# google-research/frame-interpolation

Hardware: AMD Instinct MI355X
Metric: interpolated frames/sec @1080p (higher is better)
Workload: dtype f32; 1 GPU; 1080p_2x2: 1920x1080 pair, align 64, block_shape [2, 2] -> 4 tile(s) of 960x576 in one batch, film_net published config, seeded synthetic weights, t=0.5; parallelism=1 independent GPU(s), weights RCCL-broadcast once, exec=direct launches, two lanes, lanes=1

## Files before the change

frame-interpolation_amd/csrc/conv_igemm.hip:

```cpp
#include "conv_buf_impl.h"
#include "conv_wino43_impl.h"
#include "conv_wino2d_impl.h"
#include "conv_fold4_impl.h"
#include "conv_c3_impl.h"
#ifdef FILM_EXTRA_FAMILIES
#include "conv_halo_impl.h"
#include "conv_split_impl.h"
#include "conv_wino_impl.h"
#include "conv_winox3_impl.h"
#include "conv_foldx3_impl.h"
#endif

template <int F>
static hipError_t launch_shape(const ConvParams& p, int shape, hipStream_t s) {
  switch (shape) {
    case TILE_128x128: return conv_buf_launch<128, 128, 2, 2, F>(p, s);
    case TILE_256x64: return conv_buf_launch<256, 64, 4, 1, F>(p, s);
    case TILE_256x32: return conv_buf_launch<256, 32, 4, 1, F>(p, s);
    case TILE_64x64: return conv_buf_launch<64, 64, 2, 2, F>(p, s);
    case TILE_128x32: return conv_buf_launch<128, 32, 4, 1, F>(p, s);
    case TILE_128x64: return conv_buf_launch<128, 64, 2, 2, F>(p, s);
    case TILE_256x128: return conv_buf_launch<256, 128, 4, 2, F>(p, s);
    default: return hipErrorInvalidValue;
  }
// ... 33 lines not shown

template <int F>
static hipError_t launch_wino(const ConvParams& p, int shape, hipStream_t s) {
  switch (shape) {
    case WINO_4x128: return conv_wino_launch<4, 128, 4, 2, F>(p, s);
    case WINO_4x64: return conv_wino_launch<4, 64, 4, 1, F>(p, s);
    case WINO_4x128_W16: return conv_wino_launch<4, 128, 4, 4, F>(p, s);
    case WINO_4x32: return conv_wino_launch<4, 32, 4, 1, F>(p, s);
    case WINO_8x64_W16: return conv_wino_launch<8, 64, 8, 2, F>(p, s);
    case WINO_8x32_W8: return conv_wino_launch<8, 32, 8, 1, F>(p, s);
    case WINO_2x64: return conv_wino_launch<2, 64, 2, 2, F>(p, s);
    case WINO_4x64_W8: return conv_wino_launch<4, 64, 4, 2, F>(p, s);
    default: return hipErrorInvalidValue;
  }
}

#endif

template <int F>
static hipError_t launch_wino43(const ConvParams& p, int shape, hipStream_t s) {
  switch (shape) {
    case W43_Q16_4x64_T21_P2: return conv_wino43_launch<4, 64, 2, 1, F | W43_F_PF2, 16>(p, s);
    case W43_Q16_4x32_T11_P2: return conv_wino43_launch<4, 32, 1, 1, F | W43_F_PF2, 16>(p, s);
    case W43_Q16_4x64_N1_P2: return conv_wino43_launch<4, 64, 1, 1, F | W43_F_PF2, 16, 1>(p, s);
    case W43_Q8_8x64_T21_P2: return conv_wino43_launch<8, 64, 2, 1, F | W43_F_PF2, 8>(p, s);
    case W43_Q8_8x64_N1_P2: return conv_wino43_launch<8, 64, 1, 1, F | W43_F_PF2, 8, 1>(p, s);
    case W43_Q8_8x32_T11_BG: return conv_wino43_launch<8, 32, 1, 1, F | W43_F_BG, 8>(p, s);
    case W43_Q8_8x32_T11_P2: return conv_wino43_launch<8, 32, 1, 1, F | W43_F_PF2, 8>(p, s);
#ifdef FILM_EXTRA_FAMILIES
    case W43_4x64_T21: return conv_wino43_launch<4, 64, 2, 1, F>(p, s);
    case W43_4x64_T12: return conv_wino43_launch<4, 64, 1, 2, F>(p, s);
    case W43_4x32_T11: return conv_wino43_launch<4, 32, 1, 1, F>(p, s);
    case W43_Q16_4x64_T21: return conv_wino43_launch<4, 64, 2, 1, F, 16>(p, s);
    case W43_Q16_4x64_T12: return conv_wino43_launch<4, 64, 1, 2, F, 16>(p, s);
    case W43_Q16_4x32_T11: return conv_wino43_launch<4, 32, 1, 1, F, 16>(p, s);
    case W43_Q16_4x64_N1: return conv_wino43_launch<4, 64, 1, 1, F, 16, 1>(p, s);
    case W43_Q16_4x64_T12_P2: return conv_wino43_launch<4, 64, 1, 2, F | W43_F_PF2, 16>(p, s);
    case W43_Q16_4x32_T11_BG: return conv_wino43_launch<4, 32, 1, 1, F | W43_F_BG, 16>(p, s);
    case W43_Q8_8x64_T12_P2: return conv_wino43_launch<8, 64, 1, 2, F | W43_F_PF2, 8>(p, s);
#endif
    default: return hipErrorInvalidValue;
  }
}

template <int F>
static hipError_t launch_wino2d(const ConvParams& p, int shape, hipStream_t s) {
  switch (shape) {
    case W2D_8x64: return conv_wino2d_launch_any<64, F>(p, s);
    case W2D_8x32: return conv_wino2d_launch_any<32, F>(p, s);
    case W2D_8x32_S2: return conv_wino2d_launch_any<32, F, 2>(p, s);
    case W2D_16x64: return conv_wino2d_launch_any<64, F | W2D_F_SQ>(p, s);
    case W2D_16x32: return conv_wino2d_launch_any<32, F | W2D_F_SQ>(p, s);
    case W2D_16x32_S2: return conv_wino2d_launch_any<32, F | W2D_F_SQ, 2>(p, s);
    default: return hipErrorInvalidValue;
  }
}

template <int F>
static hipError_t launch_fold4(const ConvParams& p, int shape, hipStream_t s) {
  switch (shape) {
    case F4_4x64: return conv_fold4_launch<2, F>(p, s);
    case F4_4x32: return conv_fold4_launch<1, F>(p, s);
    default: return hipErrorInvalidValue;
  }
}

#ifdef FILM_EXTRA_FAMILIES
template <int F>
static hipError_t launch_winox3(const ConvParams& p, int shape, hipStream_t s) {
  switch (shape) {
    case WX3_4x128_T22: return conv_winox3_launch<4, 128, 2, 2, F>(p, s);
    case WX3_4x64_T12: return conv_winox3_launch<4, 64, 1, 2, F>(p, s);
    case WX3_4x64_T21: return conv_winox3_launch<4, 64, 2, 1, F>(p, s);
    case WX3_4x32_T11: return conv_winox3_launch<4, 32, 1, 1, F>(p, s);
    default: return hipErrorInvalidValue;
  }
}

template <int F>
static hipError_t launch_foldx3(const ConvParams& p, int shape, hipStream_t s) {
  switch (shape) {
    case FX3_4x64: return conv_foldx3_launch<4, 64, 4, 1, F>(p, s);
    case FX3_8x64: return conv_foldx3_launch<8, 64, 8, 1, F>(p, s);
    case FX3_4x128: return conv_foldx3_launch<4, 128, 4, 2, F>(p, s);
    default: return hipErrorInvalidValue;
  }
}
#endif


__global__ __launch_bounds__(256) void conv_splitk_reduce_kernel(const float* __restrict__ part, const float* __restrict__ bias,
                                                                 float* __restrict__ out, int M, int Cout, int ostride,
                                                                 int S, int leaky) {
  const int G = Cout >> 2;
  const unsigned idx = blockIdx.x * 256u + threadIdx.x;
  if (idx >= (unsigned)M * (unsigned)G) return;
  const unsigned m = idx / (unsigned)G, g = idx - m * (unsigned)G;
  const size_t plane = (size_t)M * Cout;
  const float4* src = reinterpret_cast<const float4*>(part + (size_t)m * Cout + g * 4);
  float4 a = *reinterpret_cast<const float4*>(bias + g * 4);
  for (int sidx = 0; sidx < S; ++sidx) {
    const float4 v = src[(size_t)sidx * (plane >> 2)];
    a.x += v.x; a.y += v.y; a.z += v.z; a.w += v.w;
  }
  if (leaky) {
    a.x = a.x > 0.f ? a.x : 0.2f * a.x; a.y = a.y > 0.f ? a.y : 0.2f * a.y;
// ... 60 lines not shown
```

frame-interpolation_amd/csrc/conv_wino2d_impl.h:

```cpp
#pragma once
#include "conv_common.h"

enum { W2D_F_SQ = 128,
       W2D_F_XEPI = 8,
       W2D_DBG_TIME = 8192 };


template <bool SQ> struct W2dSlotTable { unsigned v[24 * 64]; };
template <bool SQ> constexpr W2dSlotTable<SQ> w2d_make_slot_table() {
  constexpr int QW = SQ ? 4 : 8, TH = SQ ? 16 : 8, HR = TH + 2, PW = 4 * QW + 2;
  constexpr int CO4 = (PW + 3) / 4, MO4 = 4 * CO4, RP4 = 4 * MO4 + (SQ ? 2 : 4);
  W2dSlotTable<SQ> t{};
  for (int sl = 0; sl < 24 * 64; ++sl) {
    const int r = sl / RP4, rem = sl % RP4, m = rem / MO4, rr = rem % MO4, c = rr / CO4, k = rr % CO4, px = 4 * k + m;
    const bool ok = r < HR && rem < 4 * MO4 && px < PW;
    t.v[sl] = ok ? ((unsigned)r << 24 | (unsigned)px << 8 | (unsigned)c << 4) : 0xFFFFFFFFu;
  }
  return t;
}
template <bool SQ> __device__ const W2dSlotTable<SQ> w2d_slot_table = w2d_make_slot_table<SQ>();

template <int BN, int FLAGS, int NS_ = 3>
__global__ __launch_bounds__(4 * (BN / 32) * 64, (BN == 32) ? 2 : 1) void conv_wino2d_kernel(ConvParams p) {
  constexpr bool SQ = (FLAGS & W2D_F_SQ) != 0;
  constexpr int QW = SQ ? 4 : 8, TH = SQ ? 16 : 8, HR = TH + 2, PXW = 4 * QW, PW = PXW + 2;
  static_assert(QW * (TH / 2) == 32, "32 units per tile");
  constexpr int NG = BN / 32, NW = 4 * NG;
  constexpr int CO4 = (PW + 3) / 4, MO4 = 4 * CO4, RP4 = 4 * MO4 + (SQ ? 2 : 4);
  constexpr int NREQ = 24;
  constexpr int STAGE4 = NREQ * 64;
  constexpr int NS = NS_;
  static_assert(NS == 2 || NS == 3, "stages");
  constexpr int IPW = NREQ / NW;
  static_assert(NREQ % NW == 0, "requests per wave");
  static_assert(HR * RP4 <= STAGE4, "stage size");
  constexpr bool XE = (FLAGS & W2D_F_XEPI) != 0;
  constexpr unsigned OOB = 0xFFFFFFFFu;

  extern __shared__ __attribute__((aligned(1024))) float smem[];

  const int t = threadIdx.x;
  const int lane = t & 63;
  const int wv = __builtin_amdgcn_readfirstlane(t >> 6);
  const int l31 = lane & 31, half = lane >> 5;
  const int mu = wv & 3, ng = wv >> 2;

  unsigned long long tm0 = 0, tm1 = 0, tm2 = 0, tmA = 0, tmB = 0, tmC = 0, tmW = 0, tmE1 = 0, tmE2 = 0, tmE3 = 0;
  unsigned long long rt0 = 0;
  if constexpr ((FLAGS & W2D_DBG_TIME) != 0) { rt0 = __builtin_amdgcn_s_memrealtime(); tm0 = __builtin_readcyclecounter(); }

  int aH = p.H, aW = p.W, aNB = p.NB, aCtot = p.Ctot, aKsplit = p.ksplit, aNseg = p.nseg, aUnused = p.unused_chain;
  unsigned a_tpi = p.mg_tpi, a_ntx = p.mg_ntx, a_nby = p.mg_nby;
  int ntx_ = p.tl_ntx, tpi_ = p.tl_tpi;
  int aGx = (int)gridDim.x, aGy = (int)gridDim.y;
  const float* aS0ptr = p.seg[0].ptr;
  int aS0stride = p.seg[0].stride, aS0C = p.seg[0].C, aS0boff = p.seg[0].boff, aS0bmod = p.seg[0].bmod;
  const float* aWptr = p.w;
  unsigned rtab[(24 / (4 * (BN / 32)))];
#pragma unroll
  for (int n = 0; n < 24 / NW; ++n) rtab[n] = w2d_slot_table<SQ>.v[t + 64 * NW * n];
  {
    unsigned long long q0 = (unsigned long long)(uintptr_t)aS0ptr, q1 = (unsigned long long)(uintptr_t)aWptr;
    asm volatile("" : "+s"(aH), "+s"(aW), "+s"(aNB), "+s"(aCtot), "+s"(aKsplit), "+s"(aNseg), "+s"(aUnused), "+s"(a_tpi), "+s"(a_ntx), "+s"(a_nby), "+s"(ntx_), "+s"(tpi_),
                      "+s"(aGx), "+s"(aGy), "+s"(q0), "+s"(q1), "+s"(aS0stride), "+s"(aS0C), "+s"(aS0boff), "+s"(aS0bmod));
    aS0ptr = reinterpret_cast<const float*>((uintptr_t)q0);
    aWptr = reinterpret_cast<const float*>((uintptr_t)q1);
  }
  unsigned long long tmK = 0, tmT = 0;
  if constexpr ((FLAGS & W2D_DBG_TIME) != 0) tmK = __builtin_readcyclecounter();
  int bx = blockIdx.x, by = blockIdx.y;
  if constexpr ((FLAGS & CONV_B_XCD_M) != 0) {
    const int nbx = aGx, nby = aGy;
    const int nwg = nbx * nby;
    const int lin = by * nbx + bx;
    const int xcd = lin & 7, idx = lin >> 3;
    const int q = nwg >> 3, r = nwg & 7;
    const int base = xcd < r ? xcd * (q + 1) : r * (q + 1) + (xcd - r) * q;
    const int nl = base + idx;
    bx = (int)conv_udiv((unsigned)nl, a_nby);
    by = nl - bx * nby;
  }
  const int ntx = ntx_, tpi = tpi_;
  const int img = (int)conv_udiv((unsigned)bx, a_tpi);
  const int trow0 = (int)conv_udiv((unsigned)(bx - img * tpi), a_ntx);
  const int y0 = trow0 * TH, x0 = (bx - img * tpi - trow0 * ntx) * PXW;
  const int n0 = by * BN;

  unsigned rvoff[IPW];
  int rsg = 0, rc0 = 0, rsegC = 0;
// ... 36 lines not shown
      rvoff[n] = tv == OOB ? OOB : off;
    }
  };
  auto raw_setup_seg = [&]() {
    const ConvSeg& s = p.seg[rsg];
    raw_setup_seg_of(s.ptr, s.stride, s.C, s.boff, s.bmod);
  };
  auto dma_piece = [&](int n, int stage) {
    const unsigned so = (unsigned)rc0 * 4u;
    const unsigned base = lds0 + (unsigned)stage * (STAGE4 * 16u) + (unsigned)(wv + NW * n) * 1024u;
    asm volatile("s_mov_b32 m0, %0\n\ts_nop 0\n\tbuffer_load_dwordx4 %1, %2, %3 offen lds" ::"s"(base), "v"(rvoff[n]), "s"(rrsrc), "s"(so)
                 : "memory");
  };
  auto dma_advance = [&]() {
    rc0 += 16;
    if (rc0 >= rsegC) {
      if (rsg + 1 < aNseg) { rc0 = 0; ++rsg; raw_setup_seg(); }
    }
  };
  const int ksp = XE && aKsplit > 1 ? aKsplit : 1;
  const int nsc_all = aCtot >> 4;
  int sc0 = 0, sc1 = nsc_all;
  if (ksp > 1) {
    sc0 = (int)((unsigned)nsc_all * blockIdx.z / (unsigned)ksp);
    sc1 = (int)((unsigned)nsc_all * (blockIdx.z + 1u) / (unsigned)ksp);
    int c = sc0 * 16;
    while (rsg + 1 < aNseg && c >= p.seg[rsg].C) { c -= p.seg[rsg].C; ++rsg; }
    rc0 = c;
  }
  auto raw_issue = [&](int stage) {
#pragma unroll
    for (int n = 0; n < IPW; ++n) dma_piece(n, stage);
    dma_advance();
  };

  const int nkc = aCtot / 8, nsc = sc1 - sc0, kc0 = 2 * sc0, kc1 = 2 * sc1;
  const conv_rsrc_t brsrc = conv_make_rsrc(conv_uniform_ptr(aWptr));
  const unsigned bvoff = (unsigned)((half * 32 + l31) * 16);
  const int ct = n0 / 32 + ng;
  auto slab = [&](int kc) { return (unsigned)(((ct * nkc + (kc < nkc ? kc : nkc - 1)) * 4 + mu) * 6) * 1024u; };
  bf4 fbg[2][6];

  f32x16 acc[6];

  const bf4* const smem4 = reinterpret_cast<const bf4*>(smem);
  const int ur = l31 / QW, lq = l31 % QW;
  const int ra = mu == 0 ? 0 : mu == 2 ? 2 : 1, rb = mu == 0 ? 2 : mu == 1 ? 2 : mu == 2 ? 1 : 3;
  const float sgn = mu == 1 ? 1.f : -1.f;
  const int ix_a = (2 * ur + ra) * RP4 + half * CO4 + lq, ix_b = (2 * ur + rb) * RP4 + half * CO4 + lq;
  typedef float f2 __attribute__((ext_vector_type(2)));
  f2 A[2][6][2];
  bf4 d[6];
  bf4 d2[6];

  using C0 = std::integral_constant<int, 0>;
  using C1 = std::integral_constant<int, 1>;
  auto read_row = [&](bf4 (&dst)[6], int ix, int stage, auto h_c) {
    constexpr int IMM = decltype(h_c)::value * 2 * CO4;
    const int ixs = ix + stage * STAGE4;
#pragma unroll
    for (int j = 0; j < 6; ++j) dst[j] = smem4[ixs + IMM + (j & 3) * MO4 + (j >> 2)];
  };
  auto pair_of = [](const bf4& v, int q) -> f2 { return q ? f2{v[2], v[3]} : f2{v[0], v[1]}; };
  auto set_pair = [](bf4& v, int q, f2 x) { if (q) { v[2] = x[0]; v[3] = x[1]; } else { v[0] = x[0]; v[1] = x[1]; } };
  auto fma2 = [](float k, f2 x, f2 y) -> f2 {
    f2 r;
    const f2 kk = {k, k};
    asm("v_pk_fma_f32 %0, %1, %2, %3" : "=v"(r) : "s"(kk), "v"(x), "v"(y));
    return r;
  };
  auto add2 = [](f2 x, f2 y) -> f2 { f2 r; asm("v_pk_add_f32 %0, %1, %2" : "=v"(r) : "v"(x), "v"(y)); return r; };
  auto mul2 = [](float k, f2 x) -> f2 {
    f2 r;
    const f2 kk = {k, k};
    asm("v_pk_mul_f32 %0, %1, %2" : "=v"(r) : "s"(kk), "v"(x));
    return r;
  };
  auto max1 = [](float x, float y) -> float { float r; asm("v_max_f32 %0, %1, %2" : "=v"(r) : "v"(x), "v"(y)); return r; };
  auto sub2 = [](f2 x, f2 y) -> f2 { f2 r; asm("v_pk_add_f32 %0, %1, %2 neg_lo:[0,1] neg_hi:[0,1]" : "=v"(r) : "v"(x), "v"(y)); return r; };
  f2 xt[4];
  auto xf_t = [&](int q) {
    const f2 d1 = pair_of(d[1], q), d2v = pair_of(d[2], q), d3 = pair_of(d[3], q), d4 = pair_of(d[4], q);
    xt[0] = fma2(-4.f, d2v, d4);
    xt[1] = fma2(-4.f, d1, d3);
    xt[2] = sub2(d4, d2v);
    xt[3] = sub2(d3, d1);
  };
  auto xf_v = [&](int q, int nu) -> f2 {
    switch (nu) {
      case 0: return fma2(4.f, pair_of(d[0], q), fma2(-5.f, pair_of(d[2], q), pair_of(d[4], q)));
      case 1: return add2(xt[0], xt[1]);
      case 2: return sub2(xt[0], xt[1]);
      case 3: return fma2(2.f, xt[3], xt[2]);
      case 4: return fma2(-2.f, xt[3], xt[2]);
      default: return fma2(4.f, pair_of(d[1], q), fma2(-5.f, pair_of(d[3], q), pair_of(d[5], q)));
    }
  };
  auto pin = [](f2& v) { asm volatile("" : "+v"(v)); };
  auto prepare = [&](f2 (&An)[6][2], int stage, auto h_c) {
    read_row(d, ix_a, stage, h_c);
    read_row(d2, ix_b, stage, h_c);
#pragma unroll
    for (int j = 0; j < 6; ++j)
#pragma unroll
      for (int q = 0; q < 2; ++q) set_pair(d[j], q, fma2(sgn, pair_of(d2[j], q), pair_of(d[j], q)));
#pragma unroll
    for (int q = 0; q < 2; ++q) {
      xf_t(q);
#pragma unroll
      for (int nu = 0; nu < 6; ++nu) An[nu][q] = xf_v(q, nu);
    }
  };

  if (ksp > 1) raw_setup_seg();
  else raw_setup_seg_of(aS0ptr, aS0stride, aS0C, aS0boff, aS0bmod);
  raw_issue(0);
  if constexpr ((FLAGS & W2D_DBG_TIME) != 0) tmA = __builtin_readcyclecounter();
#pragma unroll
  for (int j = 0; j < 6; ++j) fbg[0][j] = conv_buf_load(brsrc, bvoff, slab(kc0) + (unsigned)j * 1024u);
  __builtin_amdgcn_sched_barrier(0);
  asm volatile("s_waitcnt vmcnt(6)" ::: "memory");
  if constexpr ((FLAGS & W2D_DBG_TIME) != 0) tmB = __builtin_readcyclecounter();
  __syncthreads();
  if constexpr ((FLAGS & W2D_DBG_TIME) != 0) tmC = __builtin_readcyclecounter();
#pragma unroll
  for (int j = 0; j < 6; ++j) fbg[1][j] = conv_buf_load(brsrc, bvoff, slab(kc0 + 1) + (unsigned)j * 1024u);
  __builtin_amdgcn_sched_barrier(0);
  if (nsc > 1) raw_issue(1);
  if constexpr (NS > 2) { if (nsc > 2) raw_issue(2); }
  prepare(A[0], 0, C0{});

  int st_s = 0, st_n = 1;
  int st_dma = 0;
  bool dma_on = false;
  int gs = 0;
  constexpr int P1 = NS == 2 ? IPW : (IPW + 1) / 2, P0 = IPW - P1;
  auto dma_slot = [](int g, int cnt) constexpr -> int {
    if (cnt <= 0) return -1;
    if (cnt == 6) return g == 2 ? 0 : (g >= 5 && (g - 5) % 4 == 0) ? 1 + (g - 5) / 4 : -1;
    const int step = 24 / cnt, at = cnt == 1 ? 13 : 5;
    return (g % step == at && g / step < cnt) ? g / step : -1;
  };
  auto chunk = [&](int kc, auto h_c, auto first_c, auto last_c) {
    constexpr int H = decltype(h_c)::value;
    constexpr bool FIRST = decltype(first_c)::value != 0;
    constexpr bool LAST = decltype(last_c)::value != 0;
    constexpr bool PREP = !(LAST && H == 1);
    using RH = std::integral_constant<int, 1 - H>;
    const int rs = H == 0 ? st_s : st_n;
    f2(&Ac)[6][2] = A[H];
    f2(&An)[6][2] = A[1 - H];
    if constexpr (H == 1 && !LAST) {
      unsigned long long tw0 = 0;
      if constexpr ((FLAGS & W2D_DBG_TIME) != 0) tw0 = __builtin_readcyclecounter();
      if (NS == 2 || gs == 0) asm volatile("s_waitcnt vmcnt(6)" ::: "memory");
      else asm volatile("s_waitcnt vmcnt(12)" ::: "memory");
      __syncthreads();
      if constexpr ((FLAGS & W2D_DBG_TIME) != 0) tmW += __builtin_readcyclecounter() - tw0;
      dma_on = (kc >> 1) + NS < sc1;
      st_dma = st_s;
    }
    const unsigned so2 = LAST ? 0u : slab(kc + 2);
    __builtin_amdgcn_sched_barrier(0);
    auto gap = [&](auto g_c) {
      constexpr int g = decltype(g_c)::value;
      constexpr int jp = g >> 3, i8 = g & 7, k = i8 >> 1, j = 2 * jp + (i8 & 1);
      if constexpr (FIRST && k == 0) {
        const f32x16 zero = {0.f, 0.f, 0.f, 0.f, 0.f, 0.f, 0.f, 0.f, 0.f, 0.f, 0.f, 0.f, 0.f, 0.f, 0.f, 0.f};
        acc[j] = __builtin_amdgcn_mfma_f32_32x32x2f32(fbg[H][j][k], Ac[j][k >> 1][k & 1], zero, 0, 0, 0);
      } else {
        acc[j] = __builtin_amdgcn_mfma_f32_32x32x2f32(fbg[H][j][k], Ac[j][k >> 1][k & 1], acc[j], 0, 0, 0);
      }
      if constexpr (!LAST) {
        if constexpr (k == 3) fbg[H][j] = conv_buf_load(brsrc, bvoff, so2 + (unsigned)j * 1024u);
      }
      if constexpr (PREP) {
        if constexpr (g == 0) read_row(d, ix_a, rs, RH{});
        if constexpr (g == 1) read_row(d2, ix_b, rs, RH{});
        if constexpr (g >= 4 && g < 10) {
          constexpr int jj = g - 4;
#pragma unroll
          for (int q = 0; q < 2; ++q) { f2 v = fma2(sgn, pair_of(d2[jj], q), pair_of(d[jj], q)); pin(v); set_pair(d[jj], q, v); }
        }
        if constexpr (g >= 10 && g < 16) {
          constexpr int q = (g - 10) / 3, part = (g - 10) % 3;
          if constexpr (part == 0) {
            xf_t(q);
            pin(xt[0]); pin(xt[1]); pin(xt[2]); pin(xt[3]);
          } else if constexpr (part == 1) {
            An[0][q] = xf_v(q, 0);
            An[5][q] = xf_v(q, 5);
            pin(An[0][q]); pin(An[5][q]);
          } else {
#pragma unroll
            for (int nu = 1; nu < 5; ++nu) { An[nu][q] = xf_v(q, nu); pin(An[nu][q]); }
          }
        }
      }
      if constexpr (!LAST) {
        constexpr int CNT = H == 1 ? P1 : P0, N0 = H == 1 ? 0 : P1;
        constexpr int idx = dma_slot(g, CNT);
        if constexpr (idx >= 0) {
          if (dma_on) {
            dma_piece(N0 + idx, st_dma);
            if constexpr (N0 + idx == IPW - 1) dma_advance();
          }
        }
      }
      __builtin_amdgcn_sched_barrier(0);
    };
    conv_for_each(gap, std::make_integer_sequence<int, 24>{});
    if constexpr (H == 1) {
      st_s = st_n;
      st_n = st_n + 1 == NS ? 0 : st_n + 1;
      ++gs;
    }
  };

  auto epilogue = [&]() {
    const int t = threadIdx.x, lane = t & 63, l31 = lane & 31, half = lane >> 5;
    __syncthreads();
    if constexpr ((FLAGS & W2D_DBG_TIME) != 0) tmE1 = __builtin_readcyclecounter();
    float o[4][16];
  #pragma unroll
    for (int r = 0; r < 16; ++r) {
      const float m0 = acc[0][r], m1 = acc[1][r], m2 = acc[2][r], m3 = acc[3][r], m4 = acc[4][r], m5 = acc[5][r];
      const float s34 = m3 + m4, d34 = m3 - m4, d12 = m1 - m2, s12 = m1 + m2;
      o[0][r] = ((m0 + m1) + m2) + s34;
      o[1][r] = __builtin_fmaf(2.f, d34, d12);
      o[2][r] = __builtin_fmaf(4.f, s34, s12);
      o[3][r] = d12 + __builtin_fmaf(8.f, d34, m5);
    }
    bf4* const xb = reinterpret_cast<bf4*>(smem);
    constexpr int XB4 = NG * 4 * 256;
    static_assert(2 * XB4 <= NS * STAGE4, "exchange buffers");
    const int widx = (ng * 4 + mu) * 256 + l31 * 8;
    const int rng = t >> 8, run = (t >> 3) & 31, rcg = t & 7;
    const int ridx = rng * 1024 + run * 8 + (rcg ^ (run & 7));
    const int nrd = n0 + rng * 32 + rcg * 4;
    const bool rawsum = XE && ksp > 1;
    const bool has_pw = XE && p.pw_out != nullptr;
    float b0 = 0.f, b1 = 0.f, b2 = 0.f, b3 = 0.f;
    if (!rawsum) { const float* const bp = p.bias + nrd; b0 = bp[0]; b1 = bp[1]; b2 = bp[2]; b3 = bp[3]; }
    const int oy = y0 + 2 * (run / QW), ox = x0 + 4 * (run % QW);
    const int ostr = rawsum ? p.Cout : p.ostride;
    const float slope = (p.leaky && !rawsum) ? 0.2f : 1.f;
    const int dyo = 2 * (run / QW), dxo = 4 * (run % QW), nth = rng * 32 + rcg * 4;
    const int cpix = (img * p.H + y0) * p.W + x0;
    float* obase = p.out;
    if (rawsum) { asm volatile(""); obase = p.part + (size_t)blockIdx.z * p.M * p.Cout; }
    float* const ocorner = obase + ((long long)cpix * ostr + n0);
    float* const orow = ocorner + (__umul24(__umul24(dyo, p.W) + dxo, ostr) + nth);
    float* pool_base = nullptr;
    if (XE && p.pool_out) {
      asm volatile("");
      const int ppix = (img * (p.H >> 1) + (y0 >> 1)) * (p.W >> 1) + (x0 >> 1);
      pool_base = p.pool_out + ((long long)ppix * p.pool_ostride + n0) + (__umul24(__umul24(dyo >> 1, p.W >> 1) + (dxo >> 1), p.pool_ostride) + nth);
    }
    constexpr int PWS = 68;
    float* const pwt = smem + 2 * XB4 * 4;
    float* const pww = pwt + TH * PXW * PWS;
    if (has_pw && t < 256) pww[t] = (t & 3) < p.pw_cout ? p.pw_w[(t >> 2) * p.pw_cout + (t & 3)] : 0.f;
    bf4 k0 = {0.f, 0.f, 0.f, 0.f}, k1 = {0.f, 0.f, 0.f, 0.f};
    auto write_round = [&](int jx, bf4* xw) {
  #pragma unroll
      for (int g = 0; g < 4; ++g) {
        bf4 v;
        v[0] = o[jx][4 * g]; v[1] = o[jx][4 * g + 1]; v[2] = o[jx][4 * g + 2]; v[3] = o[jx][4 * g + 3];
        xw[widx + ((2 * g + half) ^ (l31 & 7))] = v;
      }
    };
  #pragma unroll
    for (int jx = 0; jx < 4; ++jx) {
      bf4* const xw = xb + (jx & 1) * XB4;
      write_round(jx, xw);
      __syncthreads();
      if constexpr ((FLAGS & W2D_DBG_TIME) != 0) { if (jx == 0) tmE2 = __builtin_readcyclecounter(); if (jx == 3) tmE3 = __builtin_readcyclecounter(); }
      const bf4 m0 = xw[ridx], m1 = xw[ridx + 256], m2 = xw[ridx + 512], m3 = xw[ridx + 768];
      bf4 r0, r1;
  #pragma unroll
      for (int q = 0; q < 2; ++q) {
        const f2 bq = q ? f2{b2, b3} : f2{b0, b1};
        const f2 v0 = add2(add2(add2(pair_of(m0, q), pair_of(m1, q)), pair_of(m2, q)), bq);
        const f2 v1 = add2(sub2(sub2(pair_of(m1, q), pair_of(m2, q)), pair_of(m3, q)), bq);
        const f2 s0 = mul2(slope, v0), s1 = mul2(slope, v1);
        set_pair(r0, q, f2{max1(v0[0], s0[0]), max1(v0[1], s0[1])});
        set_pair(r1, q, f2{max1(v1[0], s1[0]), max1(v1[1], s1[1])});
      }
// ... 25 lines not shown
        const int y = y0 + t / PXW, x = x0 + (t % PXW);
        float a[4] = {0.f, 0.f, 0.f, 0.f};
        const bf4* row = reinterpret_cast<const bf4*>(pwt + t * PWS);
        const bf4* wq = reinterpret_cast<const bf4*>(pww);
  #pragma unroll 4
        for (int c4 = 0; c4 < 16; ++c4) {
          const bf4 v = row[c4];
  #pragma unroll
          for (int k = 0; k < 4; ++k) {
            const bf4 w = wq[c4 * 4 + k];
  #pragma unroll
            for (int j = 0; j < 4; ++j) a[j] = __builtin_fmaf(v[k], w[j], a[j]);
          }
        }
        if (y < p.H && x < p.W) {
          float* dd = p.pw_out + (((size_t)img * p.H + y) * p.W + x) * p.pw_ostride;
  #pragma unroll
          for (int j = 0; j < 4; ++j)
            if (j < p.pw_cout) dd[j] = a[j] + p.pw_bias[j];
        }
      }
    }
  };
  if constexpr ((FLAGS & W2D_DBG_TIME) != 0) tm1 = __builtin_readcyclecounter();
  for (int tile = 0; tile < 1; ++tile) {
    chunk(kc0, C0{}, C1{}, C0{});
    chunk(kc0 + 1, C1{}, C0{}, C0{});
    for (int kc = kc0 + 2; kc < kc1 - 2; kc += 2) {
      chunk(kc, C0{}, C0{}, C0{});
      chunk(kc + 1, C1{}, C0{}, C0{});
    }
    if (nsc > 1) {
      chunk(kc1 - 2, C0{}, C0{}, C1{});
      chunk(kc1 - 1, C1{}, C0{}, C1{});
    }
    if constexpr ((FLAGS & W2D_DBG_TIME) != 0) tm2 = __builtin_readcyclecounter();
    epilogue();
  }
  if constexpr ((FLAGS & W2D_DBG_TIME) != 0) {
    const unsigned long long tm3 = __builtin_readcyclecounter();
    if (t == 0) {
      unsigned long long* o8 = reinterpret_cast<unsigned long long*>(p.part) + (size_t)(blockIdx.y * gridDim.x + blockIdx.x) * 16;
      o8[0] = tm0; o8[1] = tm1; o8[2] = tm2; o8[3] = tm3; o8[4] = tmA; o8[5] = tmB; o8[6] = tmC; o8[7] = tmW;
      o8[8] = rt0; o8[9] = __builtin_amdgcn_s_memrealtime();
      o8[10] = (unsigned long long)__builtin_amdgcn_s_getreg((31 << 11) | 4) | ((unsigned long long)__builtin_amdgcn_s_getreg((31 << 11) | 20) << 32);
      o8[11] = tmE1; o8[12] = tmE2; o8[13] = tmE3; o8[14] = tmK; o8[15] = tmT;
    }
  }
}

template <int BN, int FLAGS, int NS = 3>
hipError_t conv_wino2d_launch(const ConvParams& p, hipStream_t s) {
  if (!(FLAGS & W2D_F_XEPI) && (p.ksplit > 1 || p.pool_out || p.pw_out)) return hipErrorInvalidValue;
  const size_t lds = p.pw_out ? (size_t)2 * (BN / 32) * 16 * 1024 + 256 * 68 * 4 + 1024 : (size_t)NS * 24 * 1024;
  constexpr int NT = 4 * (BN / 32) * 64;
  if (p.ksize != 3 || p.Ctot % 16 || p.Cout % BN) return hipErrorInvalidValue;
  if (p.ksplit > 1 && (!p.part || (reinterpret_cast<uintptr_t>(p.part) & 15) || p.Cout % 4 || p.pool_out || p.pw_out || p.ksplit > p.Ctot / 16)) return hipErrorInvalidValue;
  if (p.pw_out) {
    if (BN != 64 || p.Cout != 64 || p.pool_out || p.pw_cout < 1 || p.pw_cout > 4) return hipErrorInvalidValue;
  } else if (p.ostride % 4 || (reinterpret_cast<uintptr_t>(p.out) & 15)) return hipErrorInvalidValue;
  if (p.pool_out && ((p.H | p.W) & 1 || p.pool_ostride % 4 || (reinterpret_cast<uintptr_t>(p.pool_out) & 15))) return hipErrorInvalidValue;
  {
    long long nimg = p.NB;
    for (int i = 0; i < p.nseg; ++i) nimg = std::max<long long>(nimg, (long long)p.seg[i].bmod);
    if ((nimg + 1) * p.H * p.W >= (1ll << 31)) return hipErrorInvalidValue;
  }
  if (p.W <= 0 || p.H <= 0 || p.W >= (1 << 20) || p.ostride >= (1 << 22) || p.pool_ostride >= (1 << 22) || p.Cout >= (1 << 22) ||
      (long long)8 * p.W * (p.ostride > p.Cout ? p.ostride : p.Cout) >= (1ll << 31)) return hipErrorInvalidValue;
  for (int i = 0; i < p.nseg; ++i)
    if ((long long)p.W * p.seg[i].stride * 4 >= (1ll << 24) || p.seg[i].C % 16 || p.seg[i].stride % 4 || p.seg[i].stride <= 0 || p.seg[i].stride >= (1 << 22) || p.seg[i].up || (reinterpret_cast<uintptr_t>(p.seg[i].ptr) & 15)) return hipErrorInvalidValue;
  constexpr bool SQ = (FLAGS & W2D_F_SQ) != 0;
  const int ntx = SQ ? (p.W + 15) / 16 : (p.W + 31) / 32, nty = SQ ? (p.H + 15) / 16 : (p.H + 7) / 8;
  const int ntiles = p.NB * ntx * nty;
  dim3 grid((unsigned)ntiles, p.Cout / BN, (unsigned)(p.ksplit > 1 ? p.ksplit : 1));
  ConvParams q = p;
  bool exact = true;
  q.mg_nby = conv_magic(grid.y, (unsigned long long)grid.x * grid.y, exact);
  q.mg_tpi = conv_magic((unsigned long long)ntx * nty, (unsigned long long)ntiles + 1, exact);
  q.mg_ntx = conv_magic(ntx, (unsigned long long)ntx * nty, exact);
  q.tl_ntx = ntx; q.tl_tpi = ntx * nty;
  if (!exact) return hipErrorInvalidValue;
  return conv_launch<conv_wino2d_kernel<BN, FLAGS, NS>>(grid, dim3(NT), lds, s, q, 144 * 1024);
}

template <int BN, int FLAGS, int NS = 3>
hipError_t conv_wino2d_launch_any(const ConvParams& p, hipStream_t s) {
  if (p.ksplit > 1 || p.pool_out || p.pw_out) return conv_wino2d_launch<BN, FLAGS | W2D_F_XEPI, NS>(p, s);
  return conv_wino2d_launch<BN, FLAGS, NS>(p, s);
}
```

frame-interpolation_amd/csrc/film_kernels.h:

```cpp
#pragma once
#include <hip/hip_runtime.h>
#include <stdint.h>

#include <vector>

#include "../../include/film_hip.h"

#define FILM_MAX_SEG 4
#define FILM_BK 16

struct ConvSeg {
  const float* ptr;
  int stride;
  int C;
  int boff, bmod;
  int up;
};

struct ConvParams {
  ConvSeg seg[FILM_MAX_SEG];
  int nseg;
  int ksize;
  const float* w;
  const float* bias;
// ... 95 lines not shown
  const float* bflow;
  const float* fflow;
  float* dst;
  int dstride;
  int64_t npix;
};

struct TileMapParams {
  const float* src;
  float* dst;
  int B, H, W;
  int bh, bw;
  int ph, pw;
  int TH, TW;
  int oy, ox;
  int tile0, ntiles;
  int ovy, ovx;
  int eh, ew;
};
__host__ __device__ inline int film_tile_origin(int i, int p, int o, int n, int e) {
  const int s = i * p - o;
  return s < 0 ? 0 : (s > n - e ? n - e : s);
}

enum ConvTile { TILE_128x128 = 0, TILE_256x64 = 1, TILE_256x32 = 2, TILE_64x64 = 3, TILE_128x32 = 4,
                TILE_128x64 = 5, TILE_256x128 = 6 , TILE_SHAPES = 7,
                TILE_C3_DIRECT = 7 , CONV_TILE_XCD = 16,
                CONV_TILE_C3 = 32 ,
                CONV_TILE_HALO = 64 ,
                CONV_TILE_WINO = 256 ,
                CONV_TILE_SPLIT = 128 ,
                CONV_TILE_X3 = 512 ,
                CONV_TILE_F43 = 2048 ,
                CONV_TILE_W2D = 8192 ,
                CONV_TILE_EXT = 4096 ,
                CONV_TILE_FOLD4 = 16384 ,
                CONV_TILE_FOLDX3 = 1024  };
enum Wino43Tile { W43_4x64_T21 = 0, W43_4x64_T12 = 1, W43_4x32_T11 = 2, W43_Q16_4x64_T21 = 3, W43_Q16_4x64_T12 = 4, W43_Q16_4x32_T11 = 5,
                  W43_Q16_4x64_N1 = 6 ,
                  W43_Q16_4x64_T21_P2 = 7, W43_Q16_4x64_T12_P2 = 8, W43_Q16_4x32_T11_P2 = 9, W43_Q16_4x64_N1_P2 = 10,
                  W43_Q16_4x32_T11_BG = 11,
                  W43_Q8_8x64_T21_P2 = 12, W43_Q8_8x64_N1_P2 = 13, W43_Q8_8x32_T11_BG = 14, W43_Q8_8x64_T12_P2 = 15,
                  W43_Q8_8x32_T11_P2 = 16 };
#ifdef FILM_EXTRA_FAMILIES
constexpr bool kExtraFamilies = true;
#else
constexpr bool kExtraFamilies = false;
#endif
static inline bool film_w43_shape_built(int sh) {
  if (kExtraFamilies) return sh >= 0 && sh <= W43_Q8_8x32_T11_P2;
  return sh == W43_Q16_4x64_T21_P2 || sh == W43_Q16_4x32_T11_P2 || sh == W43_Q16_4x64_N1_P2 || sh == W43_Q8_8x64_T21_P2 || sh == W43_Q8_8x64_N1_P2 ||
         sh == W43_Q8_8x32_T11_BG || sh == W43_Q8_8x32_T11_P2;
}
enum Wino2dTile { W2D_8x64 = 0, W2D_8x32 = 1, W2D_8x32_S2 = 2, W2D_16x64 = 3, W2D_16x32 = 4, W2D_16x32_S2 = 5, W2D_SHAPES = 6 };
inline bool film_w2d_square(int shape) { return shape >= W2D_16x64 && shape <= W2D_16x32_S2; }
inline bool film_w2d_64(int shape) { return shape == W2D_8x64 || shape == W2D_16x64; }
enum Fold4Tile { F4_4x64 = 0, F4_4x32 = 1 };
enum FoldX3Tile { FX3_4x64 = 0 , FX3_8x64 = 1 , FX3_4x128 = 2  };
enum WinoX3Tile { WX3_4x128_T22 = 0, WX3_4x64_T12 = 1, WX3_4x64_T21 = 3, WX3_4x32_T11 = 4 };
enum WinoTile { WINO_4x128 = 0 , WINO_4x64 = 1 , WINO_4x128_W16 = 2 ,
                WINO_4x64_W8 = 3 , WINO_4x32 = 4 , WINO_8x64_W16 = 5 ,
                WINO_8x32_W8 = 6 , WINO_2x64 = 7 , WINO_SHAPES = 8 };
enum HaloTile { HALO_8x128 = 0 , HALO_8x64 = 1 , HALO_8x32 = 2 , HALO_4x64 = 3 ,
                HALO_4x128 = 4 , HALO_4x32 = 5 , HALO_SHAPES = 6 };

struct TileShape { int bm, bn; };
static inline TileShape film_tile_shape(int tile) {
  switch (tile & (CONV_TILE_XCD - 1)) {
    case TILE_128x128: return {128, 128};
    case TILE_256x64: return {256, 64};
    case TILE_256x32: return {256, 32};
    case TILE_64x64: return {64, 64};
    case TILE_128x64: return {128, 64};
    case TILE_256x128: return {256, 128};
    default: return {128, 32};
  }
}

enum ConvFamily { FAM_BUF , FAM_C3, FAM_W2D, FAM_W43, FAM_FOLD4 ,
                  FAM_HALO, FAM_SPLIT6, FAM_SPLIT3, FAM_WINO, FAM_WINOX3, FAM_FOLDX3 ,
                  CONV_FAMILIES };
constexpr int CONV_TILE_FAMILY = CONV_TILE_C3 | CONV_TILE_HALO | CONV_TILE_SPLIT | CONV_TILE_WINO | CONV_TILE_X3 | CONV_TILE_FOLDX3 |
                                 CONV_TILE_F43 | CONV_TILE_W2D | CONV_TILE_FOLD4;

struct ConvWeights {
  int64_t w_off = 0;
  int64_t wh_off = -1;
  int64_t ws_off = -1;
  int64_t ww_off = -1;
  int64_t wx_off = -1;
  int64_t w43_off = -1;
  int64_t w2d_off = -1;
  int64_t wfx_off = -1;
  int64_t wf4_off = -1;
};

namespace film_internal {
struct OpDesc;
std::vector<int> tile_candidates(const OpDesc&), c3_candidates(const OpDesc&), wino2d_candidates(const OpDesc&), wino43_candidates(const OpDesc&),
    fold4_candidates(const OpDesc&), halo_candidates(const OpDesc&), wino_candidates(const OpDesc&), winox3_candidates(const OpDesc&),
    foldx3_candidates(const OpDesc&);
}
struct ConvFamilyRow {
  int flags;
  int64_t ConvWeights::* weights;
  bool splitk;
  bool in_default;
  int fused_shape;
  std::vector<int> (*candidates)(const film_internal::OpDesc&);
// ... 73 lines not shown
```

frame-interpolation_amd/csrc/film_tune.cpp:

```cpp
#include "film_internal.h"

namespace film_internal {
namespace {
std::vector<int> both_maps(ConvFamily f, const std::vector<int>& shapes) {
  std::vector<int> out;
  for (int sh : shapes) { out.push_back(conv_tile(f, sh, false)); out.push_back(conv_tile(f, sh, true)); }
  return out;
}

std::string conv_signature(const OpDesc& op) {
  std::ostringstream o;
  const FamilyCodes fc = family_codes(op.family);
  o << op.NB << 'x' << op.H << 'x' << op.W << ':' << op.Cout << ':' << op.ksize << ':' << op.out.stride << ':' << fc.c3 << ':' << fc.halo << ':' << fc.split << ':' << fc.wino << ':' << op.fold << ':' << op.ksplit << ':' << (op.out2.buf >= 0) << ':' << op.pw_cout;
  for (int i = 0; i < op.nseg; ++i)
    o << '|' << op.seg[i].v.C << ',' << op.seg[i].v.stride << ',' << op.seg[i].up << ',' << op.seg[i].bmod;
  return o.str();
}
}

std::vector<int> tile_candidates(const OpDesc& op) {
  if (op.Cout % 128 == 0) return both_maps(FAM_BUF, {TILE_128x128, TILE_256x128, TILE_256x64, TILE_128x64, TILE_64x64});
  if (op.Cout % 64 == 0) return both_maps(FAM_BUF, {TILE_256x64, TILE_128x64, TILE_64x64, TILE_256x32, TILE_128x32});
  return both_maps(FAM_BUF, {TILE_256x32, TILE_128x32});
}

std::vector<int> c3_candidates(const OpDesc&) { return {conv_tile(FAM_C3, TILE_C3_DIRECT, false)}; }

std::vector<int> halo_candidates(const OpDesc& op) {
  if (op.Cout % 128 == 0) return both_maps(op.family, {HALO_4x64, HALO_4x128, HALO_8x64, HALO_8x128});
  if (op.Cout % 64 == 0) return both_maps(op.family, {HALO_4x64, HALO_8x64, HALO_4x32, HALO_8x32});
  return both_maps(op.family, {HALO_8x32, HALO_4x32});
}

std::vector<int> wino_candidates(const OpDesc& op) {
  if (op.Cout % 128 == 0) return both_maps(FAM_WINO, {WINO_4x64_W8, WINO_8x64_W16, WINO_2x64, WINO_4x128_W16, WINO_4x128});
  if (op.Cout % 64 == 0) return both_maps(FAM_WINO, {WINO_4x64_W8, WINO_8x64_W16, WINO_2x64, WINO_4x32});
  return both_maps(FAM_WINO, {WINO_4x32, WINO_8x32_W8});
}

std::vector<int> wino43_candidates(const OpDesc& op) {
  const bool pool = op.out2.buf >= 0, pw = op.pw_out.buf >= 0;
  std::vector<int> shapes;
  if (pw)
    shapes = {W43_Q16_4x64_N1, W43_Q16_4x64_N1_P2, W43_Q8_8x64_N1_P2};
  else if (op.Cout % 64 == 0)
    shapes = {W43_4x64_T21, W43_Q16_4x64_T21, W43_Q16_4x64_T12, W43_Q16_4x32_T11, W43_Q16_4x64_N1,
              W43_Q16_4x64_T21_P2, W43_Q16_4x64_T12_P2, W43_Q16_4x32_T11_P2, W43_Q16_4x64_N1_P2, W43_Q16_4x32_T11_BG,
              W43_Q8_8x64_T21_P2, W43_Q8_8x64_T12_P2, W43_Q8_8x64_N1_P2, W43_Q8_8x32_T11_BG, W43_Q8_8x32_T11_P2};
  else
    shapes = {W43_4x32_T11, W43_Q16_4x32_T11, W43_Q16_4x32_T11_P2, W43_Q16_4x32_T11_BG, W43_Q8_8x32_T11_BG, W43_Q8_8x32_T11_P2};
  std::vector<int> keep;
  for (int sh : shapes) {
    if (!film_w43_shape_built(sh)) continue;
    if (pool && (sh == W43_4x64_T21 || sh == W43_4x64_T12 || sh == W43_4x32_T11)) continue;
    keep.push_back(sh);
  }
  return both_maps(FAM_W43, keep);
}

std::vector<int> wino2d_candidates(const OpDesc& op) {
  const int H = op.H, W = op.W;
  const bool pw = op.pw_out.buf >= 0;
  const int64_t pad_r = (int64_t)((W + 31) / 32) * ((H + 7) / 8), pad_s = (int64_t)((W + 15) / 16) * ((H + 15) / 16);
  const bool sq = pad_s <= pad_r;
  std::vector<int> shapes;
  if (pw || op.Cout % 64 == 0) { shapes.push_back(W2D_8x64); if (sq) shapes.push_back(W2D_16x64); }
  if (!pw) {
    shapes.push_back(W2D_8x32); shapes.push_back(W2D_8x32_S2);
    if (sq) { shapes.push_back(W2D_16x32); shapes.push_back(W2D_16x32_S2); }
  }
  return both_maps(FAM_W2D, shapes);
}

std::vector<int> fold4_candidates(const OpDesc& op) {
  return both_maps(FAM_FOLD4, op.Cout % 64 == 0 ? std::vector<int>{F4_4x64, F4_4x32} : std::vector<int>{F4_4x32});
}

std::vector<int> foldx3_candidates(const OpDesc& op) {
  return both_maps(FAM_FOLDX3, op.Cout % 128 == 0 ? std::vector<int>{FX3_4x64, FX3_8x64, FX3_4x128} : std::vector<int>{FX3_4x64, FX3_8x64});
}

std::vector<int> winox3_candidates(const OpDesc& op) {
  if (op.Cout % 128 == 0) return both_maps(FAM_WINOX3, {WX3_4x128_T22, WX3_4x64_T12, WX3_4x64_T21});
  if (op.Cout % 64 == 0) return both_maps(FAM_WINOX3, {WX3_4x64_T12, WX3_4x64_T21, WX3_4x32_T11});
  return both_maps(FAM_WINOX3, {WX3_4x32_T11});
}

std::vector<int> conv_candidates(const OpDesc& op) { return kConvFamily[op.family].candidates(op); }

int autotune_plan(film_t* h, Plan* P, bool measure) {
  bool need = false;
  for (const OpDesc& op : P->ops) {
    if (op.kind != OP_CONV || !measure) continue;
    const std::string sig = conv_signature(op);
    if (h->tune_cache.count(sig)) continue;
    auto it = h->tune_import.find(sig);
    if (it != h->tune_import.end()) {
      const std::vector<int> cands = conv_candidates(op);
      if (std::find(cands.begin(), cands.end(), it->second) != cands.end()) { h->tune_cache[sig] = it->second; continue; }
    }
    need = true;
  }
  if (need) {
    HIPCHK(h, film_launch_fill_random(P->arena, P->arena_floats, 0x9e3779b9u, h->stream));
    hipEvent_t e0, e1;
    HIPCHK(h, hipEventCreate(&e0));
    HIPCHK(h, hipEventCreate(&e1));
    for (OpDesc& op : P->ops) {
      if (op.kind != OP_CONV) continue;
      const std::string sig = conv_signature(op);
      if (h->tune_cache.count(sig)) continue;
      int best = op.tile;
      float best_ms = 1e30f;
      const std::vector<int> cands = conv_candidates(op);
      auto launch_tile = [&](int tile) -> hipError_t {
        OpDesc trial = op;
        trial.tile = tile;
        return launch_op(trial, P->arena, h->packed_dev, h->stream);
      };
      auto time_once = [&](int tile, float* ms) -> int {
        HIPCHK(h, hipEventRecord(e0, h->stream));
        HIPCHK(h, launch_tile(tile));
        HIPCHK(h, hipEventRecord(e1, h->stream));
// ... 91 lines not shown
```

Baseline: 30.25 frames/s.

## Share Winograd input transforms across wave pairs via an LDS ring in wino2d

Adds a shared-fragment variant of the 2D Winograd conv kernel (BN=64, two raw stages). Each of the two waves per mu now transforms only half of the input pairs and writes the transformed fragments into a 4-slot LDS ring that both waves then read, which removes duplicated transform arithmetic and LDS reads. It also reorders the prologue and DMA schedule. The cost is a much larger LDS footprint (144 KB), which lowers occupancy, plus extra ring writes and reads. The new tile shapes are added as autotuner candidates, so they are only used where they win.

New measurement: 30.03 frames/s. No clear change (-0.7%).

```diff
diff --git a/frame-interpolation_amd/csrc/conv_igemm.hip b/frame-interpolation_amd/csrc/conv_igemm.hip
--- a/frame-interpolation_amd/csrc/conv_igemm.hip
+++ b/frame-interpolation_amd/csrc/conv_igemm.hip
@@ -109,6 +109,8 @@
     case W2D_16x64: return conv_wino2d_launch_any<64, F | W2D_F_SQ>(p, s);
     case W2D_16x32: return conv_wino2d_launch_any<32, F | W2D_F_SQ>(p, s);
     case W2D_16x32_S2: return conv_wino2d_launch_any<32, F | W2D_F_SQ, 2>(p, s);
+    case W2D_8x64_SH: return conv_wino2d_launch_any<64, F | W2D_F_SHF, 2>(p, s);
+    case W2D_16x64_SH: return conv_wino2d_launch_any<64, F | W2D_F_SQ | W2D_F_SHF, 2>(p, s);
     default: return hipErrorInvalidValue;
   }
 }
diff --git a/frame-interpolation_amd/csrc/conv_wino2d_impl.h b/frame-interpolation_amd/csrc/conv_wino2d_impl.h
--- a/frame-interpolation_amd/csrc/conv_wino2d_impl.h
+++ b/frame-interpolation_amd/csrc/conv_wino2d_impl.h
@@ -3,6 +3,7 @@
 
 enum { W2D_F_SQ = 128,
        W2D_F_XEPI = 8,
+       W2D_F_SHF = 256,
        W2D_DBG_TIME = 8192 };
 
 
@@ -35,6 +36,9 @@
   static_assert(NREQ % NW == 0, "requests per wave");
   static_assert(HR * RP4 <= STAGE4, "stage size");
   constexpr bool XE = (FLAGS & W2D_F_XEPI) != 0;
+  constexpr bool SHF = (FLAGS & W2D_F_SHF) != 0;
+  static_assert(!SHF || (BN == 64 && NS == 2), "shared fragments: two waves per mu, two raw stages");
+  constexpr int RING4 = NS * STAGE4, RSLOT4 = 4 * 6 * 64;
   constexpr unsigned OOB = 0xFFFFFFFFu;
 
   extern __shared__ __attribute__((aligned(1024))) float smem[];
@@ -177,6 +181,12 @@
   f2 A[2][6][2];
   bf4 d[6];
   bf4 d2[6];
+  f2 e[6], e2[6], xs[4], en[6];
+  typedef __attribute__((address_space(3))) f2 lds_f2;
+  typedef __attribute__((address_space(3))) bf4 lds_bf4;
+  const unsigned ab_a = lds0 + 16u * (unsigned)ix_a + 8u * (unsigned)ng, ab_b = lds0 + 16u * (unsigned)ix_b + 8u * (unsigned)ng;
+  const unsigned ab_r = lds0 + 16u * (unsigned)(RING4 + mu * (6 * 64) + lane);
+  int rg = 1;
 
   using C0 = std::integral_constant<int, 0>;
   using C1 = std::integral_constant<int, 1>;
@@ -237,6 +247,59 @@
     }
   };
 
+  auto read_pair_row = [&](f2 (&dst)[6], unsigned ab, int stage, auto h_c) {
+    constexpr int IMM = decltype(h_c)::value * 2 * CO4;
+    unsigned a = ab + (unsigned)stage * (STAGE4 * 16u);
+    asm volatile("" : "+v"(a));
+    const lds_f2* const q = reinterpret_cast<const lds_f2*>(a);
+#pragma unroll
+    for (int j = 0; j < 6; ++j) dst[j] = q[2 * (IMM + (j & 3) * MO4 + (j >> 2))];
+  };
+  auto ycomb = [&](int j) { e[j] = fma2(sgn, e2[j], e[j]); };
+  auto xs_t = [&](int i) {
+    switch (i) {
+      case 0: xs[0] = fma2(-4.f, e[2], e[4]); break;
+      case 1: xs[1] = fma2(-4.f, e[1], e[3]); break;
+      case 2: xs[2] = sub2(e[4], e[2]); break;
+      default: xs[3] = sub2(e[3], e[1]); break;
+    }
+  };
+  auto xs_v = [&](int nu) -> f2 {
+    switch (nu) {
+      case 0: return fma2(4.f, e[0], fma2(-5.f, e[2], e[4]));
+      case 1: return add2(xs[0], xs[1]);
+      case 2: return sub2(xs[0], xs[1]);
+      case 3: return fma2(2.f, xs[3], xs[2]);
+      case 4: return fma2(-2.f, xs[3], xs[2]);
+      default: return fma2(4.f, e[1], fma2(-5.f, e[3], e[5]));
+    }
+  };
+  unsigned ring_wa = 0;
+  auto ring_write_at = [&](int slot) { ring_wa = ab_r + 8u * (unsigned)ng + (unsigned)slot * (RSLOT4 * 16u); asm volatile("" : "+v"(ring_wa)); };
+  auto ring_write = [&](int nu) { reinterpret_cast<lds_f2*>(ring_wa)[2 * nu * 64] = en[nu]; };
+  auto ring_read = [&](f2 (&An)[6][2], int slot) {
+    unsigned a = ab_r + (unsigned)slot * (RSLOT4 * 16u);
+    asm volatile("" : "+v"(a));
+    const lds_bf4* const q = reinterpret_cast<const lds_bf4*>(a);
+#pragma unroll
+    for (int nu = 0; nu < 6; ++nu) {
+      const bf4 v = q[nu * 64];
+      An[nu][0] = f2{v[0], v[1]};
+      An[nu][1] = f2{v[2], v[3]};
+    }
+  };
+  auto prepare_pair = [&](int stage, auto h_c, int slot) {
+    read_pair_row(e, ab_a, stage, h_c);
+    read_pair_row(e2, ab_b, stage, h_c);
+    ring_write_at(slot);
+#pragma unroll
+    for (int j = 0; j < 6; ++j) ycomb(j);
+#pragma unroll
+    for (int i = 0; i < 4; ++i) xs_t(i);
+#pragma unroll
+    for (int nu = 0; nu < 6; ++nu) { en[nu] = xs_v(nu); ring_write(nu); }
+  };
+
   if (ksp > 1) raw_setup_seg();
   else raw_setup_seg_of(aS0ptr, aS0stride, aS0C, aS0boff, aS0bmod);
   raw_issue(0);
@@ -248,12 +311,27 @@
   if constexpr ((FLAGS & W2D_DBG_TIME) != 0) tmB = __builtin_readcyclecounter();
   __syncthreads();
   if constexpr ((FLAGS & W2D_DBG_TIME) != 0) tmC = __builtin_readcyclecounter();
-#pragma unroll
-  for (int j = 0; j < 6; ++j) fbg[1][j] = conv_buf_load(brsrc, bvoff, slab(kc0 + 1) + (unsigned)j * 1024u);
-  __builtin_amdgcn_sched_barrier(0);
-  if (nsc > 1) raw_issue(1);
-  if constexpr (NS > 2) { if (nsc > 2) raw_issue(2); }
-  prepare(A[0], 0, C0{});
+  if constexpr (SHF) {
+    if (nsc > 1) raw_issue(1);
+#pragma unroll
+    for (int j = 0; j < 6; ++j) fbg[1][j] = conv_buf_load(brsrc, bvoff, slab(kc0 + 1) + (unsigned)j * 1024u);
+    __builtin_amdgcn_sched_barrier(0);
+    prepare_pair(0, C0{}, 0);
+    prepare_pair(0, C1{}, 1);
+    __builtin_amdgcn_sched_barrier(0);
+    asm volatile("s_waitcnt vmcnt(6)" ::: "memory");
+    __syncthreads();
+    if (nsc > 2) raw_issue(0);
+    prepare_pair(1, C0{}, 2);
+    ring_read(A[0], 0);
+  } else {
+#pragma unroll
+    for (int j = 0; j < 6; ++j) fbg[1][j] = conv_buf_load(brsrc, bvoff, slab(kc0 + 1) + (unsigned)j * 1024u);
+    __builtin_amdgcn_sched_barrier(0);
+    if (nsc > 1) raw_issue(1);
+    if constexpr (NS > 2) { if (nsc > 2) raw_issue(2); }
+    prepare(A[0], 0, C0{});
+  }
 
   int st_s = 0, st_n = 1;
   int st_dma = 0;
@@ -272,7 +350,7 @@
     constexpr bool LAST = decltype(last_c)::value != 0;
     constexpr bool PREP = !(LAST && H == 1);
     using RH = std::integral_constant<int, 1 - H>;
-    const int rs = H == 0 ? st_s : st_n;
+    const int rs = SHF ? (H == 0 ? st_n : st_s) : (H == 0 ? st_s : st_n);
     f2(&Ac)[6][2] = A[H];
     f2(&An)[6][2] = A[1 - H];
     if constexpr (H == 1 && !LAST) {
@@ -282,8 +360,8 @@
       else asm volatile("s_waitcnt vmcnt(12)" ::: "memory");
       __syncthreads();
       if constexpr ((FLAGS & W2D_DBG_TIME) != 0) tmW += __builtin_readcyclecounter() - tw0;
-      dma_on = (kc >> 1) + NS < sc1;
-      st_dma = st_s;
+      dma_on = (kc >> 1) + (SHF ? 3 : NS) < sc1;
+      st_dma = SHF ? st_n : st_s;
     }
     const unsigned so2 = LAST ? 0u : slab(kc + 2);
     __builtin_amdgcn_sched_barrier(0);
@@ -299,7 +377,22 @@
       if constexpr (!LAST) {
         if constexpr (k == 3) fbg[H][j] = conv_buf_load(brsrc, bvoff, so2 + (unsigned)j * 1024u);
       }
-      if constexpr (PREP) {
+      if constexpr (SHF) {
+        if constexpr (PREP && g == 0) ring_read(An, rg);
+        if constexpr (!LAST) {
+          if constexpr (g == 1) read_pair_row(e, ab_a, rs, RH{});
+          if constexpr (g == 2) read_pair_row(e2, ab_b, rs, RH{});
+          if constexpr (g >= 4 && g < 10) { ycomb(g - 4); pin(e[g - 4]); }
+          if constexpr (g == 10) { xs_t(0); xs_t(1); pin(xs[0]); pin(xs[1]); }
+          if constexpr (g == 11) { xs_t(2); xs_t(3); pin(xs[2]); pin(xs[3]); }
+          if constexpr (g == 12) { en[0] = xs_v(0); pin(en[0]); }
+          if constexpr (g == 13) { en[5] = xs_v(5); pin(en[5]); }
+          if constexpr (g == 14) { en[1] = xs_v(1); en[2] = xs_v(2); pin(en[1]); pin(en[2]); }
+          if constexpr (g == 15) { en[3] = xs_v(3); en[4] = xs_v(4); pin(en[3]); pin(en[4]); }
+          if constexpr (g == 16) ring_write_at(rg ^ 2);
+          if constexpr (g >= 16 && g < 22) ring_write(g - 16);
+        }
+      } else if constexpr (PREP) {
         if constexpr (g == 0) read_row(d, ix_a, rs, RH{});
         if constexpr (g == 1) read_row(d2, ix_b, rs, RH{});
         if constexpr (g >= 4 && g < 10) {
@@ -340,6 +433,7 @@
       st_n = st_n + 1 == NS ? 0 : st_n + 1;
       ++gs;
     }
+    if constexpr (SHF) rg = (rg + 1) & 3;
   };
 
   auto epilogue = [&]() {
@@ -358,7 +452,7 @@
     }
     bf4* const xb = reinterpret_cast<bf4*>(smem);
     constexpr int XB4 = NG * 4 * 256;
-    static_assert(2 * XB4 <= NS * STAGE4, "exchange buffers");
+    static_assert(2 * XB4 <= NS * STAGE4 + (SHF ? 4 * RSLOT4 : 0), "exchange buffers");
     const int widx = (ng * 4 + mu) * 256 + l31 * 8;
     const int rng = t >> 8, run = (t >> 3) & 31, rcg = t & 7;
     const int ridx = rng * 1024 + run * 8 + (rcg ^ (run & 7));
@@ -490,7 +584,8 @@
 template <int BN, int FLAGS, int NS = 3>
 hipError_t conv_wino2d_launch(const ConvParams& p, hipStream_t s) {
   if (!(FLAGS & W2D_F_XEPI) && (p.ksplit > 1 || p.pool_out || p.pw_out)) return hipErrorInvalidValue;
-  const size_t lds = p.pw_out ? (size_t)2 * (BN / 32) * 16 * 1024 + 256 * 68 * 4 + 1024 : (size_t)NS * 24 * 1024;
+  static_assert(!(FLAGS & W2D_F_SHF) || (BN == 64 && NS == 2), "shared fragments: BN = 64, two stages");
+  const size_t lds = (FLAGS & W2D_F_SHF) ? (size_t)144 * 1024 : p.pw_out ? (size_t)2 * (BN / 32) * 16 * 1024 + 256 * 68 * 4 + 1024 : (size_t)NS * 24 * 1024;
   constexpr int NT = 4 * (BN / 32) * 64;
   if (p.ksize != 3 || p.Ctot % 16 || p.Cout % BN) return hipErrorInvalidValue;
   if (p.ksplit > 1 && (!p.part || (reinterpret_cast<uintptr_t>(p.part) & 15) || p.Cout % 4 || p.pool_out || p.pw_out || p.ksplit > p.Ctot / 16)) return hipErrorInvalidValue;
diff --git a/frame-interpolation_amd/csrc/film_kernels.h b/frame-interpolation_amd/csrc/film_kernels.h
--- a/frame-interpolation_amd/csrc/film_kernels.h
+++ b/frame-interpolation_amd/csrc/film_kernels.h
@@ -171,9 +171,10 @@
   return sh == W43_Q16_4x64_T21_P2 || sh == W43_Q16_4x32_T11_P2 || sh == W43_Q16_4x64_N1_P2 || sh == W43_Q8_8x64_T21_P2 || sh == W43_Q8_8x64_N1_P2 ||
          sh == W43_Q8_8x32_T11_BG || sh == W43_Q8_8x32_T11_P2;
 }
-enum Wino2dTile { W2D_8x64 = 0, W2D_8x32 = 1, W2D_8x32_S2 = 2, W2D_16x64 = 3, W2D_16x32 = 4, W2D_16x32_S2 = 5, W2D_SHAPES = 6 };
-inline bool film_w2d_square(int shape) { return shape >= W2D_16x64 && shape <= W2D_16x32_S2; }
-inline bool film_w2d_64(int shape) { return shape == W2D_8x64 || shape == W2D_16x64; }
+enum Wino2dTile { W2D_8x64 = 0, W2D_8x32 = 1, W2D_8x32_S2 = 2, W2D_16x64 = 3, W2D_16x32 = 4, W2D_16x32_S2 = 5, W2D_SHAPES = 6,
+                  W2D_8x64_SH = 6, W2D_16x64_SH = 7 };
+inline bool film_w2d_square(int shape) { return (shape >= W2D_16x64 && shape <= W2D_16x32_S2) || shape == W2D_16x64_SH; }
+inline bool film_w2d_64(int shape) { return shape == W2D_8x64 || shape == W2D_16x64 || shape == W2D_8x64_SH || shape == W2D_16x64_SH; }
 enum Fold4Tile { F4_4x64 = 0, F4_4x32 = 1 };
 enum FoldX3Tile { FX3_4x64 = 0 , FX3_8x64 = 1 , FX3_4x128 = 2  };
 enum WinoX3Tile { WX3_4x128_T22 = 0, WX3_4x64_T12 = 1, WX3_4x64_T21 = 3, WX3_4x32_T11 = 4 };
diff --git a/frame-interpolation_amd/csrc/film_tune.cpp b/frame-interpolation_amd/csrc/film_tune.cpp
--- a/frame-interpolation_amd/csrc/film_tune.cpp
+++ b/frame-interpolation_amd/csrc/film_tune.cpp
@@ -65,10 +65,12 @@
   const bool sq = pad_s <= pad_r;
   std::vector<int> shapes;
   if (pw || op.Cout % 64 == 0) { shapes.push_back(W2D_8x64); if (sq) shapes.push_back(W2D_16x64); }
+  const size_t n64 = shapes.size();
   if (!pw) {
     shapes.push_back(W2D_8x32); shapes.push_back(W2D_8x32_S2);
     if (sq) { shapes.push_back(W2D_16x32); shapes.push_back(W2D_16x32_S2); }
   }
+  if (n64 > 0) { shapes.push_back(W2D_8x64_SH); if (n64 > 1) shapes.push_back(W2D_16x64_SH); }
   return both_maps(FAM_W2D, shapes);
 }
 
```
